# val-iisc/Reflecting-Reality

Measured on AMD Instinct MI355X. Metric: images/sec at 512x512, 50-step DDIM, SD1.5+BrushNet, higher is better.
Workload: dtype bf16; 1 GPU; SD1.5 + BrushNet(6 cond ch) depth-cond inpaint, batch 4x512x512 per GPU, 50-step DDIM, CFG 7.5, VAE encode+decode included, random-init weights, inputs resident on the device; per_gpu_batch=4, global_batch=4, height=512, width=512, denoise_steps=50, parallelism=batch-shard x1 (no collective)

## Files before the change

### reflecting-reality_amd/csrc/gemm_conv_kernel.h

```cpp
#pragma once
#include "mf_common.h"

#include <type_traits>

#ifndef MF_XTAP
#define MF_XTAP 1
#endif
#ifndef MF_AEARLY
#define MF_AEARLY 1
#endif

namespace mfgemm {

static __device__ __attribute__((aligned(16))) unsigned int g_zero_page[16];

#ifdef MF_STAMPS
#define MF_STAMP(slot) do { if (p.stamps) { const int t_ = (int)threadIdx.x; \
    if (t_ == 0) p.stamps[(size_t)blockIdx.x * 32 + (slot)] = __builtin_amdgcn_s_memrealtime(); \
    else if (t_ == (int)blockDim.x - 256) p.stamps[(size_t)blockIdx.x * 32 + 16 + (slot)] = __builtin_amdgcn_s_memrealtime(); } } while (0)
#define MF_STAMP_DRAIN() asm volatile("s_waitcnt vmcnt(0)" ::: "memory")
#define MF_CLK(v) const unsigned long long v = __builtin_amdgcn_s_memtime()
#define MF_SUM(acc, a, b) acc += (b) - (a)
#define MF_PUT(slot, v) do { if (p.stamps) { const int t_ = (int)threadIdx.x; \
    if (t_ == 0) p.stamps[(size_t)blockIdx.x * 32 + (slot)] = (v); \
    else if (t_ == (int)blockDim.x - 256) p.stamps[(size_t)blockIdx.x * 32 + 16 + (slot)] = (v); } } while (0)
#else
#define MF_STAMP(slot) do { } while (0)
#define MF_STAMP_DRAIN() do { } while (0)
#define MF_CLK(v) do { } while (0)
#define MF_SUM(acc, a, b) do { } while (0)
#define MF_PUT(slot, v) do { } while (0)
#endif

struct GemmArgs {
    const char* a0; const char* a1;
    int C0, Ctot;
    int ld0b, ld1b;
    int Hin, Win, Ho, Wo, HoWo, KW, stride, pad_t, pad_l, ups;
    const char* w; int64_t ldw;
    int M, N, K;
    int zdiv; int64_t a_zs_o, a_zs_i, w_zs_o, w_zs_i, o_zs_o, o_zs_i;
    int splitk, kt_per_split, nkt, nz;
    float* ws;
    unsigned* sk_tickets;
    const float* bias; int bias_mode;
    const float* rs; const float* cs; int64_t rs_zs, cs_zs;
    const float* temb; int64_t ld_temb;
    const char* res0; int res0_dt; int64_t ld_res0;
    const char* res1; int res1_dt; int64_t ld_res1;
    int res1_rows;
    float alpha; int act;
    char* out; int out_dt; int64_t ldc;
    int tiles_n, tiles_m, ord_mfast, ord_pw, nblk, vec_ok, fast, dbg_no_res_pre;
    int dbg_epi;
    int pointwise;
    int howo_sh, wo_sh, ho_sh;
    unsigned wfr_magic;
    int epb;
    int epb_sh;
// ... 94 lines not shown
    if (p.act == MF_ACT_SILU) {
#pragma unroll
        for (int j = 0; j < 8; ++j) v[j] = silu_precise(v[j]);
    }
    if (p.act == MF_ACT_GEGLU4) {
        float g[4];
        if (p.out_dt != MF_F32) {
#pragma unroll
            for (int j = 0; j < 4; ++j) {
                const float x = v[4 + j];
                const float z = fabsf(x) * 0.70710678118654752440f;
                const float t = __builtin_amdgcn_rcpf(fmaf(0.3275911f, z, 1.0f));
                const float poly = t * fmaf(t, fmaf(t, fmaf(t, fmaf(t, 1.061405429f, -1.453152027f), 1.421413741f), -0.284496736f), 0.254829592f);
                const float e = 1.0f - poly * __builtin_amdgcn_exp2f(-z * z * 1.44269504088896340736f);
                g[j] = v[j] * (0.5f * x + 0.5f * fabsf(x) * e);
            }
        } else {
#pragma unroll
            for (int j = 0; j < 4; ++j) g[j] = v[j] * (0.5f * v[4 + j] * (1.0f + erff(v[4 + j] * 0.70710678118654752440f)));
        }
        const int64_t o = zo + (int64_t)m * p.ldc + (n >> 1);
        if (p.out_dt == MF_F32) {
            *reinterpret_cast<float4*>(p.out + o * 4) = make_float4(g[0], g[1], g[2], g[3]);
        } else {
            uint2 u;
            u.x = pack_h2<F16>(g[0], g[1]);
            u.y = pack_h2<F16>(g[2], g[3]);
            *reinterpret_cast<uint2*>(p.out + o * 2) = u;
        }
        return;
    }
    const int64_t o = zo + (int64_t)m * p.ldc + n;
    if (p.out_dt == MF_F32) {
        *reinterpret_cast<float4*>(p.out + o * 4) = make_float4(v[0], v[1], v[2], v[3]);
        *reinterpret_cast<float4*>(p.out + o * 4 + 16) = make_float4(v[4], v[5], v[6], v[7]);
    } else {
        *reinterpret_cast<uint4*>(p.out + o * 2) = pack_h8<F16>(v);
    }
}

__device__ __forceinline__ uint4 ld8f_to_bf16(const char* p) {
    const float4 lo = *reinterpret_cast<const float4*>(p);
    const float4 hi = *reinterpret_cast<const float4*>(p + 16);
    uint4 r;
    r.x = pack_bf16x2(lo.x, lo.y);
    r.y = pack_bf16x2(lo.z, lo.w);
    r.z = pack_bf16x2(hi.x, hi.y);
    r.w = pack_bf16x2(hi.z, hi.w);
    return r;
}

typedef __attribute__((address_space(1))) const void* gbl_ptr_t;

__device__ __forceinline__ void dma16(const char* src, char* lds_wave_base) {
    const unsigned lds_off = __builtin_amdgcn_readfirstlane((unsigned)(size_t)(lds_ptr_t)lds_wave_base);
    unsigned keep;
    asm volatile("s_mov_b32 %0, m0\n\ts_mov_b32 m0, %2\n\ts_nop 0\n\tglobal_load_lds_dwordx4 %1, off\n\ts_mov_b32 m0, %0"
                 : "=&s"(keep) : "v"(src), "s"(lds_off) : "memory");
}

template <int DT>
__device__ __forceinline__ f32x4_t mfma16x32(bf16x8_t a, bf16x8_t b, f32x4_t c, int, int, int) {
    if constexpr (DT == MF_F16) return __builtin_amdgcn_mfma_f32_16x16x32_f16(__builtin_bit_cast(f16x8_t, a), __builtin_bit_cast(f16x8_t, b), c, 0, 0, 0);
    else return __builtin_amdgcn_mfma_f32_16x16x32_bf16(a, b, c, 0, 0, 0);
}
template <int DT>
__device__ __forceinline__ f32x16_t mfma32x16(bf16x8_t a, bf16x8_t b, f32x16_t c) {
    if constexpr (DT == MF_F16) return __builtin_amdgcn_mfma_f32_32x32x16_f16(__builtin_bit_cast(f16x8_t, a), __builtin_bit_cast(f16x8_t, b), c, 0, 0, 0);
    else return __builtin_amdgcn_mfma_f32_32x32x16_bf16(a, b, c, 0, 0, 0);
}

#define MF_FX_XT 1
#define MF_FX_EPB 2
#define MF_FX_AE 4
#define MF_FX_ALL 7
#define MF_FX_XQ 8

constexpr int epb_pitch(int bn) { return (bn + 63) / 64 * 64; }
constexpr int epb_off(int bm, int bn, int stages, bool dx, bool ws) {
    return dx ? 2 * (bm + 32) * 128 + (ws ? stages : 2) * bn * 128 : stages * (bm + bn) * 128 + (ws ? bm * 8 : 0);
}
constexpr int epb_nimg(int bm, int bn, int stages, bool dx, bool ws) {
    if (!ws) return 0;
    const int room = 160 * 1024 - epb_off(bm, bn, stages, dx, ws), row = epb_pitch(bn) * 4;
    return room >= 6 * row ? 4 : (room >= 3 * row ? 1 : 0);
}

constexpr int min_waves(int bm, int bn, int stages, int nthr) {
    const int smem = stages * (bm + bn) * 128;
    int blocks = 160 * 1024 / smem;
    if (blocks > 8) blocks = 8;
    int w = blocks * (nthr / 64) / 4;
    return w < 1 ? 1 : (w > 4 ? 4 : w);
}

template <int BM, int BN, int NT_ALL, bool F16>
__device__ __forceinline__ void splitk_combine_tail(const GemmArgs& p, char* smem, int tile_m, int tile_n, int z, int zq, int64_t zo, int t) {
    asm volatile("s_waitcnt vmcnt(0)" ::: "memory");
    __syncthreads();
    unsigned* last_flag = reinterpret_cast<unsigned*>(smem);
    if (t == 0) {
        __builtin_amdgcn_fence(__ATOMIC_RELEASE, "agent");
        asm volatile("s_waitcnt vmcnt(0)" ::: "memory");
        unsigned* tk = p.sk_tickets + ((int64_t)z * p.tiles_m + tile_m) * p.tiles_n + tile_n;
        const unsigned prev = __hip_atomic_fetch_add(tk, 1u, __ATOMIC_RELAXED, __HIP_MEMORY_SCOPE_AGENT);
        const bool last = prev == (unsigned)p.splitk - 1u;
// ... 298 lines not shown
    auto store_tile_regs = [&](int stage) {
        char* As = smem + stage * STAGE_BYTES + tid * 16;
        char* Bs = As + BM * 128;
#pragma unroll
        for (int i = 0; i < (A_F32 ? A_IT : 1); ++i) *reinterpret_cast<uint4*>(As + i * RPP * 128) = ra[i];
#pragma unroll
        for (int i = 0; i < (A_F32 ? B_IT : 1); ++i) *reinterpret_cast<uint4*>(Bs + i * RPP * 128) = rb[i];
    };

    f32x16_t acc[MT][NT];
#pragma unroll
    for (int i = 0; i < MT; ++i)
#pragma unroll
        for (int j = 0; j < NT; ++j)
#pragma unroll
            for (int e = 0; e < 16; ++e) acc[i][j][e] = 0.0f;
    f32x4_t acc16[P16 ? MT16 : 1][P16 ? NT16 : 1];
#pragma unroll
    for (int a = 0; a < (P16 ? MT16 : 1); ++a)
#pragma unroll
        for (int b = 0; b < (P16 ? NT16 : 1); ++b) acc16[a][b] = f32x4_t{0.0f, 0.0f, 0.0f, 0.0f};

    const int frow = lane & 31;
    const int fh = lane >> 5;
    const int fkey = (frow >> 1) & 7;

    float split_amax = 0.0f;
    auto split8 = [&](const uint4& c0, const uint4& c1, uint4& hi, uint4& lo) {
        const float x[8] = {__uint_as_float(c0.x), __uint_as_float(c0.y), __uint_as_float(c0.z), __uint_as_float(c0.w),
                            __uint_as_float(c1.x), __uint_as_float(c1.y), __uint_as_float(c1.z), __uint_as_float(c1.w)};
        if constexpr (DT == MF_F16X3) {
#pragma unroll
            for (int e = 0; e < 4; ++e) split_amax = mf_amax3(split_amax, x[2 * e], x[2 * e + 1]);
        }
        unsigned h[4], l[4];
#pragma unroll
        for (int e = 0; e < 4; ++e) {
            if constexpr (X1) {
                h[e] = pack_bf16x2(x[2 * e], x[2 * e + 1]);
                l[e] = 0;
            } else if constexpr (DT == MF_F16X3) {
                mf_split_f16x2(x[2 * e], x[2 * e + 1], h[e], l[e]);
            } else {
                const unsigned ua = __float_as_uint(x[2 * e]), ub = __float_as_uint(x[2 * e + 1]);
                h[e] = (ua >> 16) | (ub & 0xffff0000u);
                l[e] = pack_bf16x2(x[2 * e] - __uint_as_float(ua & 0xffff0000u), x[2 * e + 1] - __uint_as_float(ub & 0xffff0000u));
            }
        }
        hi = uint4{h[0], h[1], h[2], h[3]};
        lo = uint4{l[0], l[1], l[2], l[3]};
    };
    auto mma16 = [&](const uint4& a, const uint4& b, f32x16_t& c) {
        if constexpr (DT == MF_F16X3)
            c = __builtin_amdgcn_mfma_f32_32x32x16_f16(__builtin_bit_cast(f16x8_t, a), __builtin_bit_cast(f16x8_t, b), c, 0, 0, 0);
        else
            c = __builtin_amdgcn_mfma_f32_32x32x16_bf16(__builtin_bit_cast(bf16x8_t, a), __builtin_bit_cast(bf16x8_t, b), c, 0, 0, 0);
    };
    auto compute_split = [&](const char* const (&Ap)[MT], const int (&Ak)[MT], const char* Bp) {
        if constexpr (FP8) {
#pragma unroll
            for (int ks = 0; ks < 2; ++ks) {
                i32x8_t fa[MT], fb[NT];
#pragma unroll
                for (int i = 0; i < MT; ++i) {
                    const uint4 c0 = *reinterpret_cast<const uint4*>(Ap[i] + (((4 * ks + 2 * fh) ^ Ak[i]) << 4));
                    const uint4 c1 = *reinterpret_cast<const uint4*>(Ap[i] + (((4 * ks + 2 * fh + 1) ^ Ak[i]) << 4));
                    fa[i] = i32x8_t{(int)c0.x, (int)c0.y, (int)c0.z, (int)c0.w, (int)c1.x, (int)c1.y, (int)c1.z, (int)c1.w};
                }
#pragma unroll
                for (int j = 0; j < NT; ++j) {
                    const uint4 c0 = *reinterpret_cast<const uint4*>(Bp + j * 32 * 128 + (((4 * ks + 2 * fh) ^ fkey) << 4));
                    const uint4 c1 = *reinterpret_cast<const uint4*>(Bp + j * 32 * 128 + (((4 * ks + 2 * fh + 1) ^ fkey) << 4));
                    fb[j] = i32x8_t{(int)c0.x, (int)c0.y, (int)c0.z, (int)c0.w, (int)c1.x, (int)c1.y, (int)c1.z, (int)c1.w};
                }
#pragma unroll
                for (int i = 0; i < MT; ++i)
#pragma unroll
                    for (int j = 0; j < NT; ++j)
                        acc[i][j] = __builtin_amdgcn_mfma_scale_f32_32x32x64_f8f6f4(fa[i], fb[j], acc[i][j], 0, 0, 0, 0x7f7f7f7f, 0, 0x7f7f7f7f);
            }
            return;
        }
#pragma unroll
        for (int ks = 0; ks < 2; ++ks) {
            uint4 ah[MT], al[MT], bh[NT], bl[NT];
#pragma unroll
            for (int i = 0; i < MT; ++i) {
                const uint4 c0 = *reinterpret_cast<const uint4*>(Ap[i] + (((4 * ks + 2 * fh) ^ Ak[i]) << 4));
                const uint4 c1 = *reinterpret_cast<const uint4*>(Ap[i] + (((4 * ks + 2 * fh + 1) ^ Ak[i]) << 4));
                split8(c0, c1, ah[i], al[i]);
            }
#pragma unroll
            for (int j = 0; j < NT; ++j) {
                if constexpr (WPK) {
                    bh[j] = *reinterpret_cast<const uint4*>(Bp + j * 32 * 128 + (((2 * ks + fh) ^ fkey) << 4));
                    bl[j] = *reinterpret_cast<const uint4*>(Bp + j * 32 * 128 + (((4 + 2 * ks + fh) ^ fkey) << 4));
                } else {
                    const uint4 c0 = *reinterpret_cast<const uint4*>(Bp + j * 32 * 128 + (((4 * ks + 2 * fh) ^ fkey) << 4));
                    const uint4 c1 = *reinterpret_cast<const uint4*>(Bp + j * 32 * 128 + (((4 * ks + 2 * fh + 1) ^ fkey) << 4));
                    split8(c0, c1, bh[j], bl[j]);
                }
            }
#pragma unroll
            for (int i = 0; i < MT; ++i)
#pragma unroll
                for (int j = 0; j < NT; ++j) {
                    if constexpr (!X1) {
                        mma16(al[i], bh[j], acc[i][j]);
                        mma16(ah[i], bl[j], acc[i][j]);
                    }
                    mma16(ah[i], bh[j], acc[i][j]);
                }
        }
    };

    const int r16 = lane & 15, kg = lane >> 4;
    auto compute_m16 = [&](const char* const (&Ap)[2 * MT], const int (&Ak)[2 * MT], const char* Bp) {
        const int key16 = (r16 >> 1) & 7;
        uint4 fa[2][2 * MT], fb[2][2 * NT];
#pragma unroll
        for (int ks = 0; ks < 2; ++ks) {
#pragma unroll
            for (int t = 0; t < 2 * MT; ++t) fa[ks][t] = *reinterpret_cast<const uint4*>(Ap[t] + (((4 * ks + kg) ^ Ak[t]) << 4));
#pragma unroll
            for (int t = 0; t < 2 * NT; ++t) fb[ks][t] = *reinterpret_cast<const uint4*>(Bp + t * 16 * 128 + (((4 * ks + kg) ^ key16) << 4));
        }
#pragma unroll
        for (int ks = 0; ks < 2; ++ks)
#pragma unroll
            for (int i = 0; i < MT; ++i)
#pragma unroll
                for (int j = 0; j < NT; ++j)
#pragma unroll
                    for (int q = 0; q < 4; ++q) {
                        f32x4_t c = {acc[i][j][4 * q], acc[i][j][4 * q + 1], acc[i][j][4 * q + 2], acc[i][j][4 * q + 3]};
                        c = mfma16x32<DT>(__builtin_bit_cast(bf16x8_t, fa[ks][2 * i + (q >> 1)]),
                                                                    __builtin_bit_cast(bf16x8_t, fb[ks][2 * j + (q & 1)]), c, 0, 0, 0);
                        acc[i][j][4 * q] = c[0]; acc[i][j][4 * q + 1] = c[1]; acc[i][j][4 * q + 2] = c[2]; acc[i][j][4 * q + 3] = c[3];
                    }
    };

    auto mma = [&](const uint4 (&fa)[MT], const uint4 (&fb)[NT]) {
#pragma unroll
        for (int i = 0; i < MT; ++i)
#pragma unroll
            for (int j = 0; j < NT; ++j) {
                if constexpr (DT == MF_BF16) {
                    acc[i][j] = __builtin_amdgcn_mfma_f32_32x32x16_bf16(
                        __builtin_bit_cast(bf16x8_t, fa[i]), __builtin_bit_cast(bf16x8_t, fb[j]), acc[i][j], 0, 0, 0);
                } else if constexpr (DT == MF_F16) {
                    acc[i][j] = __builtin_amdgcn_mfma_f32_32x32x16_f16(
                        __builtin_bit_cast(f16x8_t, fa[i]), __builtin_bit_cast(f16x8_t, fb[j]), acc[i][j], 0, 0, 0);
                } else {
                    const f32x4_t av = __builtin_bit_cast(f32x4_t, fa[i]);
                    const f32x4_t bv = __builtin_bit_cast(f32x4_t, fb[j]);
#pragma unroll
                    for (int e = 0; e < 4; ++e)
                        acc[i][j] = __builtin_amdgcn_mfma_f32_32x32x2f32(av[e], bv[e], acc[i][j], 0, 0, 0);
                }
            }
    };
    auto compute = [&](int stage) {
        if constexpr (P16) {
            const char* A16 = smem + stage * STAGE_BYTES + (wm * WM + r16) * 128;
            const char* B16 = smem + stage * STAGE_BYTES + BM * 128 + (wn * WN + r16) * 128;
            const int key16 = (r16 >> 1) & 7;
            uint4 fa[2][MT16], fb[2][NT16];
#pragma unroll
            for (int ks = 0; ks < 2; ++ks) {
#pragma unroll
                for (int t = 0; t < MT16; ++t) fa[ks][t] = *reinterpret_cast<const uint4*>(A16 + t * 16 * 128 + (((4 * ks + kg) ^ key16) << 4));
#pragma unroll
                for (int b = 0; b < NT16; ++b) fb[ks][b] = *reinterpret_cast<const uint4*>(B16 + b * 16 * 128 + (((4 * ks + kg) ^ key16) << 4));
            }
#pragma unroll
            for (int ks = 0; ks < 2; ++ks)
#pragma unroll
                for (int a = 0; a < MT16; ++a)
#pragma unroll
                    for (int b = 0; b < NT16; ++b)
                        acc16[a][b] = mfma16x32<DT>(__builtin_bit_cast(bf16x8_t, fa[ks][a]),
                                                                              __builtin_bit_cast(bf16x8_t, fb[ks][b]), acc16[a][b], 0, 0, 0);
            return;
        }
        const char* As = smem + stage * STAGE_BYTES + (wm * WM + frow) * 128;
        const char* Bs = smem + stage * STAGE_BYTES + BM * 128 + (wn * WN + frow) * 128;
        if constexpr (SPLIT || FP8) {
            const char* Ap[MT]; int Ak[MT];
#pragma unroll
            for (int i = 0; i < MT; ++i) { Ap[i] = As + i * 32 * 128; Ak[i] = fkey; }
            compute_split(Ap, Ak, Bs);
            return;
        }
        if constexpr (M16) {
            const char* A16 = smem + stage * STAGE_BYTES + (wm * WM + r16) * 128;
            const char* B16 = smem + stage * STAGE_BYTES + BM * 128 + (wn * WN + r16) * 128;
            const char* Ap[2 * MT]; int Ak[2 * MT];
#pragma unroll
            for (int t = 0; t < 2 * MT; ++t) { Ap[t] = A16 + t * 16 * 128; Ak[t] = (r16 >> 1) & 7; }
            compute_m16(Ap, Ak, B16);
            return;
        }
        uint4 fa0[MT], fb0[NT], fa1[MT], fb1[NT];
        auto ldfrag = [&](int ks, uint4 (&fa)[MT], uint4 (&fb)[NT]) {
            const int coff = (((2 * ks + fh) ^ fkey) << 4);
#pragma unroll
            for (int i = 0; i < MT; ++i) fa[i] = *reinterpret_cast<const uint4*>(As + i * 32 * 128 + coff);
#pragma unroll
            for (int j = 0; j < NT; ++j) fb[j] = *reinterpret_cast<const uint4*>(Bs + j * 32 * 128 + coff);
        };
        ldfrag(0, fa0, fb0);
        ldfrag(1, fa1, fb1);
        __builtin_amdgcn_sched_barrier(0);
        mma(fa0, fb0);
        __builtin_amdgcn_sched_barrier(0);
        ldfrag(2, fa0, fb0);
        __builtin_amdgcn_sched_barrier(0);
        mma(fa1, fb1);
        __builtin_amdgcn_sched_barrier(0);
        ldfrag(3, fa1, fb1);
        __builtin_amdgcn_sched_barrier(0);
        mma(fa0, fb0);
        mma(fa1, fb1);
    };

    constexpr bool XQ = (FX & MF_FX_XQ) != 0 && WS && H16 && !A_F32 && !M16 && !P16;
    constexpr bool XT = XQ || ((FX & MF_FX_XT) != 0 && WS && H16 && !A_F32 && (MF_XTAP != 0) && !(WAVES_M == 8 && WAVES_N == 1));
    constexpr int XNA = !XT ? 1 : XQ ? MT : (P16 ? MT16 : 2 * MT), XNB = !XT ? 1 : XQ ? NT : (P16 ? NT16 : 2 * NT);
    uint4 xa[2][XNA], xb[2][XNB];
    auto xt_load = [&](auto S, auto P, const char* Ab, auto arow, const char* Bb) {
        constexpr int ss = decltype(S)::value, hh = decltype(P)::value;
        if constexpr (XQ) {
            const int ch = 2 * hh + fh;
#pragma unroll
            for (int i = 0; i < MT; ++i) {
                const int r = arow(i);
                xa[ss][i] = *reinterpret_cast<const uint4*>(Ab + r * 128 + ((ch ^ ((r >> 1) & 7)) << 4));
            }
#pragma unroll
            for (int j = 0; j < NT; ++j) xb[ss][j] = *reinterpret_cast<const uint4*>(Bb + j * 32 * 128 + ((ch ^ fkey) << 4));
        } else if constexpr (P16 || M16) {
            const int key16 = (r16 >> 1) & 7;
#pragma unroll
            for (int t = 0; t < XNA; ++t) {
                const int r = arow(t);
                xa[ss][t] = *reinterpret_cast<const uint4*>(Ab + r * 128 + (((4 * hh + kg) ^ ((r >> 1) & 7)) << 4));
            }
#pragma unroll
            for (int t = 0; t < XNB; ++t) xb[ss][t] = *reinterpret_cast<const uint4*>(Bb + t * 16 * 128 + (((4 * hh + kg) ^ key16) << 4));
        } else {
#pragma unroll
            for (int kk = 0; kk < 2; ++kk) {
                const int ch = 2 * (2 * hh + kk) + fh;
#pragma unroll
                for (int i = 0; i < MT; ++i) {
                    const int r = arow(i);
                    xa[ss][kk * MT + i] = *reinterpret_cast<const uint4*>(Ab + r * 128 + ((ch ^ ((r >> 1) & 7)) << 4));
                }
#pragma unroll
                for (int j = 0; j < NT; ++j) xb[ss][kk * NT + j] = *reinterpret_cast<const uint4*>(Bb + j * 32 * 128 + ((ch ^ fkey) << 4));
            }
        }
    };
    auto xt_mma = [&](auto S) {
        constexpr int hh = decltype(S)::value;
        if constexpr (XQ) {
#pragma unroll
            for (int i = 0; i < MT; ++i)
#pragma unroll
                for (int j = 0; j < NT; ++j)
                    acc[i][j] = mfma32x16<DT>(__builtin_bit_cast(bf16x8_t, xa[hh][i]), __builtin_bit_cast(bf16x8_t, xb[hh][j]), acc[i][j]);
        } else if constexpr (P16) {
#pragma unroll
            for (int a = 0; a < MT16; ++a)
#pragma unroll
                for (int b = 0; b < NT16; ++b)
                    acc16[a][b] = mfma16x32<DT>(__builtin_bit_cast(bf16x8_t, xa[hh][a]),
                                                                          __builtin_bit_cast(bf16x8_t, xb[hh][b]), acc16[a][b], 0, 0, 0);
        } else if constexpr (M16) {
#pragma unroll
            for (int i = 0; i < MT; ++i)
#pragma unroll
                for (int j = 0; j < NT; ++j)
#pragma unroll
                    for (int q = 0; q < 4; ++q) {
                        f32x4_t c = {acc[i][j][4 * q], acc[i][j][4 * q + 1], acc[i][j][4 * q + 2], acc[i][j][4 * q + 3]};
                        c = mfma16x32<DT>(__builtin_bit_cast(bf16x8_t, xa[hh][2 * i + (q >> 1)]),
                                                                    __builtin_bit_cast(bf16x8_t, xb[hh][2 * j + (q & 1)]), c, 0, 0, 0);
                        acc[i][j][4 * q] = c[0]; acc[i][j][4 * q + 1] = c[1]; acc[i][j][4 * q + 2] = c[2]; acc[i][j][4 * q + 3] = c[3];
                    }
        } else {
#pragma unroll
            for (int kk = 0; kk < 2; ++kk)
#pragma unroll
                for (int i = 0; i < MT; ++i)
#pragma unroll
                    for (int j = 0; j < NT; ++j)
                        acc[i][j] = mfma32x16<DT>(__builtin_bit_cast(bf16x8_t, xa[hh][kk * MT + i]), __builtin_bit_cast(bf16x8_t, xb[hh][kk * NT + j]), acc[i][j]);
        }
    };
    using H0 = std::integral_constant<int, 0>;
    using H1 = std::integral_constant<int, 1>;
    using H2 = std::integral_constant<int, 2>;
    using H3 = std::integral_constant<int, 3>;
    auto xt_loop = [&](auto&& ld, auto&& adv) {
        auto head = [&]() {
            ld(H1{}, H1{});
            __builtin_amdgcn_sched_barrier(0);
            xt_mma(H0{});
            __builtin_amdgcn_sched_barrier(0);
            if constexpr (XQ) {
                ld(H0{}, H2{});
                __builtin_amdgcn_sched_barrier(0);
                xt_mma(H1{});
                __builtin_amdgcn_sched_barrier(0);
                ld(H1{}, H3{});
                __builtin_amdgcn_sched_barrier(0);
                xt_mma(H0{});
                __builtin_amdgcn_sched_barrier(0);
            }
        };
        ld(H0{}, H0{});
        [[maybe_unused]] unsigned long long w_bar = 0;
        MF_CLK(tl0);
        for (int t = 0; t + 1 < nt; ++t) {
            head();
            adv();
            __builtin_amdgcn_s_waitcnt(0xc07f);
            MF_CLK(tb0);
            __builtin_amdgcn_s_barrier();
            MF_CLK(tb1);
            MF_SUM(w_bar, tb0, tb1);
            ld(H0{}, H0{});
            __builtin_amdgcn_sched_barrier(0);
            xt_mma(H1{});
            __builtin_amdgcn_sched_barrier(0);
        }
        head();
        xt_mma(H1{});
        MF_CLK(tl1);
        MF_PUT(13, w_bar); MF_PUT(14, tl1 - tl0); MF_PUT(15, (unsigned long long)nt);
    };

    MF_STAMP(1);
    if (nt > 0) {
        if constexpr (DXR) {
            static_assert(!A_F32 && (WS ? STAGES == 3 : STAGES == 2), "dx reuse: DMA staging; W ring 2 deep, 3 when WS (a 4-deep ring measured no faster)");
            constexpr int WST = WS ? STAGES : 2;
            constexpr int AROWS = BM + RPP, A3_IT = AROWS / RPP;
            constexpr int AB = AROWS * 128, WB = BN * 128;
            static_assert(WAVES_M * WAVES_N * SR * EP_RS <= 2 * AB + WST * WB, "epilogue slabs must fit in this loop's LDS");
// ... 54 lines not shown
#pragma unroll
                for (int i = 0; i < B_IT; ++i) dma16_buf(w3[i] + wk, sW, lb + i * RPP * 128);
                if (AE && i_kx == 2 && i_tap + 1 < nt) {
                    int n_cg = i_cg + 1, n_ky = i_ky;
                    if (n_cg == nck) { n_cg = 0; ++n_ky; }
                    issue_a(n_ky, n_cg, i_grp + 1);
                }
                ++i_tap;
                if (++i_kx == 3) {
                    i_kx = 0; ++i_grp;
                    if (++i_cg == nck) { i_cg = 0; ++i_ky; }
                }
            };
            int arow0[MT];
#pragma unroll
            for (int i = 0; i < MT; ++i) {
                const int m = wm * WM + i * 32 + frow;
                const int ir = p.wo_sh >= 0 ? m >> weff_sh : m / weff;
                arow0[i] = ir * wfr + (m - ir * weff);
            }
            int arow16[2 * MT];
#pragma unroll
            for (int t = 0; t < 2 * MT; ++t) {
                const int m = wm * WM + t * 16 + r16;
                const int ir = p.wo_sh >= 0 ? m >> weff_sh : m / weff;
                arow16[t] = ir * wfr + (m - ir * weff);
            }
            auto compute3 = [&](int abuf, int wstage, int kx) {
                const char* Ab = smem + abuf * AB;
                if constexpr (P16) {
                    const char* Bp = smem + 2 * AB + wstage * WB + (wn * WN + r16) * 128;
                    const int key16 = (r16 >> 1) & 7;
                    const char* Ap[MT16]; int Ak[MT16];
#pragma unroll
                    for (int t = 0; t < MT16; ++t) {
                        const int r = arow16[t] + kx;
                        Ap[t] = Ab + r * 128;
                        Ak[t] = (r >> 1) & 7;
                    }
                    uint4 fa[2][MT16], fb[2][NT16];
#pragma unroll
                    for (int ks = 0; ks < 2; ++ks) {
#pragma unroll
                        for (int t = 0; t < MT16; ++t) fa[ks][t] = *reinterpret_cast<const uint4*>(Ap[t] + (((4 * ks + kg) ^ Ak[t]) << 4));
#pragma unroll
                        for (int b = 0; b < NT16; ++b) fb[ks][b] = *reinterpret_cast<const uint4*>(Bp + b * 16 * 128 + (((4 * ks + kg) ^ key16) << 4));
                    }
#pragma unroll
                    for (int ks = 0; ks < 2; ++ks)
#pragma unroll
                        for (int a = 0; a < MT16; ++a)
#pragma unroll
                            for (int b = 0; b < NT16; ++b)
                                acc16[a][b] = mfma16x32<DT>(__builtin_bit_cast(bf16x8_t, fa[ks][a]),
                                                                                      __builtin_bit_cast(bf16x8_t, fb[ks][b]), acc16[a][b], 0, 0, 0);
                    return;
                }
                const char* Bs = smem + 2 * AB + wstage * WB + (wn * WN + frow) * 128;
                if constexpr (M16) {
                    const char* Ap[2 * MT]; int Ak[2 * MT];
#pragma unroll
                    for (int t = 0; t < 2 * MT; ++t) {
                        const int r = arow16[t] + kx;
                        Ap[t] = Ab + r * 128;
                        Ak[t] = (r >> 1) & 7;
                    }
                    compute_m16(Ap, Ak, smem + 2 * AB + wstage * WB + (wn * WN + r16) * 128);
                    return;
                }
                int aoffs[MT], akey[MT];
#pragma unroll
                for (int i = 0; i < MT; ++i) {
                    const int r = arow0[i] + kx;
                    aoffs[i] = r * 128;
                    akey[i] = (r >> 1) & 7;
                }
                if constexpr (SPLIT || FP8) {
                    const char* Ap[MT];
#pragma unroll
                    for (int i = 0; i < MT; ++i) Ap[i] = Ab + aoffs[i];
                    compute_split(Ap, akey, Bs);
                    return;
                }
                uint4 fa0[MT], fb0[NT], fa1[MT], fb1[NT];
                auto ldfrag = [&](int ks, uint4 (&fa)[MT], uint4 (&fb)[NT]) {
                    const int cb = (((2 * ks + fh) ^ fkey) << 4);
#pragma unroll
                    for (int i = 0; i < MT; ++i)
                        fa[i] = *reinterpret_cast<const uint4*>(Ab + aoffs[i] + (((2 * ks + fh) ^ akey[i]) << 4));
#pragma unroll
                    for (int j = 0; j < NT; ++j) fb[j] = *reinterpret_cast<const uint4*>(Bs + j * 32 * 128 + cb);
                };
                ldfrag(0, fa0, fb0);
                ldfrag(1, fa1, fb1);
                __builtin_amdgcn_sched_barrier(0);
                mma(fa0, fb0);
                __builtin_amdgcn_sched_barrier(0);
                ldfrag(2, fa0, fb0);
                __builtin_amdgcn_sched_barrier(0);
                mma(fa1, fb1);
                __builtin_amdgcn_sched_barrier(0);
                ldfrag(3, fa1, fb1);
                __builtin_amdgcn_sched_barrier(0);
                mma(fa0, fb0);
                mma(fa1, fb1);
            };
            if constexpr (WS) {
                constexpr int PFD = WST - 1;
// ... 189 lines not shown
                            if constexpr (P16 || M16) xt_load(S, P, Ab, [&](int t) { return arb + t * 16; }, Bb);
                            else xt_load(S, P, Ab, [&](int i) { return arb + i * 32; }, Bb);
                        };
                        xt_loop(ld, [&]() { st_c = st_c == STAGES - 1 ? 0 : st_c + 1; });
                    } else
                    for (int t = 0; t < nt; ++t) {
                        compute(st_c);
                        st_c = st_c == STAGES - 1 ? 0 : st_c + 1;
                        if (t + 1 < nt) __builtin_amdgcn_s_barrier();
                    }
                }
            };
            if constexpr (WS) {
                if (p.fast) {
                    if (producer) fast_init();
                    ring_ws(issue_tile_fast);
                } else {
                    ring_ws(issue_tile);
                }
            } else if (p.fast) {
                fast_init();
                ring(issue_tile_fast);
            } else {
                ring(issue_tile);
            }
        } else {
            load_tile_regs();
            store_tile_regs(0);
            if (nt > 1) load_tile_regs();
            __syncthreads();
            for (int t = 0; t < nt; ++t) {
                compute(t & 1);
                if (t + 1 < nt) {
                    store_tile_regs((t + 1) & 1);
                    if (t + 2 < nt) load_tile_regs();
                }
                __syncthreads();
            }
        }
    }
    MF_STAMP(3);
    if constexpr (EPB_NIMG > 0) {
        if (producer && epb) wait_vmcnt<0>();
    }
    __syncthreads();
    MF_STAMP(4);
    if constexpr (DT == MF_F16X3) mf_raise_if_over(p.ovf, split_amax);

    char* slab = smem + wave * (SR * EP_RS);
    constexpr int CPR = WN / 8;
    constexpr int ITEMS = SR * CPR;
    float* ws = p.splitk > 1 ? p.ws + ((int64_t)ksplit * p.nz + z) * (int64_t)p.M * p.N : nullptr;
    const int64_t zo = zq * p.o_zs_o + zr * p.o_zs_i;
    const bool res_pre = !ws && p.vec_ok && (p.res0 || p.res1) && (!p.res0 || p.res0_dt != MF_F32) &&
                         (!p.res1 || p.res1_dt != MF_F32) && !p.dbg_no_res_pre;
    constexpr int NIT = (ITEMS + 63) / 64;
    if constexpr (WS) {
        constexpr int NCW = WAVES_M * WAVES_N, TW = NCW + 4, NCHUNK = NCW * NIT, MAXC = (NCHUNK + TW - 1) / TW;
        const int g = producer ? NCW + wave : wave;
        const bool gn = p.gn_part != nullptr;
        constexpr int GNP = (NCW * WN + TW * 64 - 1) / (TW * 64);
        float gns[GNP], gnq[GNP];
#pragma unroll
        for (int k = 0; k < GNP; ++k) { gns[k] = 0.0f; gnq[k] = 0.0f; }
#pragma unroll
        for (int ih = 0; ih < MT * (32 / SR); ++ih) {
            const int i = ih / (32 / SR), half = ih % (32 / SR);
            uint4 q0[MAXC], q1[MAXC];
            auto coords = [&](int u, int& sw, int& row, int& ec, int& m, int& n) -> bool {
                const int c = g + u * TW;
                sw = c / NIT;
                const int it = (c - sw * NIT) * 64 + lane;
                row = it / CPR; ec = (it - row * CPR) * 8;
                const int swm = sw / WAVES_N, swn = sw - swm * WAVES_N;
                m = m0 + swm * WM + i * 32 + half * SR + row;
                n = n0 + swn * WN + ec;
                return c < NCHUNK && (ITEMS % 64 == 0 || it < ITEMS);
            };
            if (res_pre) {
#pragma unroll
                for (int u = 0; u < MAXC; ++u) {
                    int sw, row, ec, m, n;
                    const bool on = coords(u, sw, row, ec, m, n);
                    q0[u] = uint4{0, 0, 0, 0}; q1[u] = uint4{0, 0, 0, 0};
                    if (on && m < p.M && n + 8 <= p.N) {
                        if (p.res0) q0[u] = *reinterpret_cast<const uint4*>(p.res0 + ((int64_t)m * p.ld_res0 + n) * 2);
                        if (p.res1) q1[u] = *reinterpret_cast<const uint4*>(p.res1 + ((int64_t)res1_row(p, m) * p.ld_res1 + n) * 2);
                    }
                }
            }
            if (!producer) {
                if constexpr (P16) {
#pragma unroll
                    for (int a = 0; a < 2; ++a)
#pragma unroll
                        for (int b = 0; b < NT16; ++b)
#pragma unroll
                            for (int r = 0; r < 4; ++r) {
                                const int row = 16 * a + 4 * kg + r - half * SR;
                                if (SR == 32 || a == half)
                                    *reinterpret_cast<float*>(slab + row * EP_RS + (16 * b + r16) * 4) = acc16[2 * i + a][b][r];
                            }
                } else {
#pragma unroll
                    for (int j = 0; j < NT; ++j)
#pragma unroll
                        for (int e = half * (SR / 2); e < half * (SR / 2) + SR / 2; ++e) {
                            if constexpr (M16) {
                                const int row = 16 * (e >> 3) + 4 * kg + (e & 3) - half * SR;
                                *reinterpret_cast<float*>(slab + row * EP_RS + (j * 32 + 16 * ((e >> 2) & 1) + r16) * 4) = acc[i][j][e];
                            } else {
                                const int row = (e & 3) + 8 * (e >> 2) + 4 * fh - half * SR;
                                *reinterpret_cast<float*>(slab + row * EP_RS + (j * 32 + frow) * 4) = acc[i][j][e];
                            }
                        }
                }
            }
            MF_STAMP(7 + 3 * ih);
            __builtin_amdgcn_s_waitcnt(0xc07f);
            __builtin_amdgcn_s_barrier();
            MF_STAMP(8 + 3 * ih);
#pragma unroll
            for (int u = 0; u < MAXC; ++u) {
                int sw, row, ec, m, n;
                if (!coords(u, sw, row, ec, m, n)) continue;
                const char* sl = smem + sw * (SR * EP_RS);
                const float2* lnst = reinterpret_cast<const float2*>(smem + STAGES * STAGE_BYTES);
                if (p.vt_out && n0 + (sw % WAVES_N) * WN >= p.vt_n0) {
                    static_assert(SR % 8 == 0 && (SR / 8) * WN == ITEMS, "transposed items cover the slab");
                    const int c = g + u * TW, it = (c - sw * NIT) * 64 + lane;
                    const int rg = it % (SR / 8), col = it / (SR / 8);
                    const int swm = sw / WAVES_N, swn = sw - swm * WAVES_N;
                    const int mt = m0 + swm * WM + i * 32 + half * SR + rg * 8, nt_ = n0 + swn * WN + col;
                    if (mt < p.M && nt_ < p.N) {
                        float tv[8];
#pragma unroll
                        for (int j = 0; j < 8; ++j) tv[j] = *reinterpret_cast<const float*>(sl + (rg * 8 + j) * EP_RS + col * 4);
                        const char* erow = smem + EPB_OFF + (nt_ - n0) * 4;
                        if (p.ln_cs) {
                            const float cs = epb ? *reinterpret_cast<const float*>(erow + EPB_PITCH * 4) : p.ln_cs[nt_];
#pragma unroll
                            for (int j = 0; j < 8; ++j) {
                                const float2 st = lnst[mt - m0 + j];
                                tv[j] = st.y * (tv[j] - st.x * cs);
                            }
                        }
                        const float b = p.bias ? (epb ? *reinterpret_cast<const float*>(erow) : p.bias[nt_]) : 0.0f;
#pragma unroll
                        for (int j = 0; j < 8; ++j) tv[j] = (tv[j] + b) * p.alpha;
                        const int img = mt / p.vt_tokens, tok = mt - img * p.vt_tokens;
                        const uint4 o = pack_h8<DT == MF_F16>(tv);
                        *reinterpret_cast<uint4*>(p.vt_out + (((int64_t)img * (p.N - p.vt_n0) + (nt_ - p.vt_n0)) * p.vt_ld + tok) * 2) = o;
                    }
                    continue;
                }
                float v[8];
                float4 lo, hi;
#ifdef MF_STAMPS
                if (p.dbg_epi & 2) { lo = make_float4(1.0f, 2.0f, 3.0f, (float)u); hi = lo; } else
#endif
                {
                    lo = *reinterpret_cast<const float4*>(sl + row * EP_RS + ec * 4);
                    hi = *reinterpret_cast<const float4*>(sl + row * EP_RS + ec * 4 + 16);
                }
#ifdef MF_STAMPS
                if (p.dbg_epi & 1) { asm volatile("" ::"v"(lo.x), "v"(hi.w)); continue; }
#endif
                if (p.ln_cs && m < p.M && n + 8 <= p.N) {
                    const float2 st = lnst[m - m0];
                    const float* lc = epb ? reinterpret_cast<const float*>(smem + EPB_OFF + (EPB_PITCH + n - n0) * 4) : p.ln_cs + n;
                    const float4 c0 = *reinterpret_cast<const float4*>(lc);
                    const float4 c1 = *reinterpret_cast<const float4*>(lc + 4);
                    lo.x = st.y * (lo.x - st.x * c0.x); lo.y = st.y * (lo.y - st.x * c0.y);
                    lo.z = st.y * (lo.z - st.x * c0.z); lo.w = st.y * (lo.w - st.x * c0.w);
                    hi.x = st.y * (hi.x - st.x * c1.x); hi.y = st.y * (hi.y - st.x * c1.y);
                    hi.z = st.y * (hi.z - st.x * c1.z); hi.w = st.y * (hi.w - st.x * c1.w);
                }
                v[0] = lo.x; v[1] = lo.y; v[2] = lo.z; v[3] = lo.w; v[4] = hi.x; v[5] = hi.y; v[6] = hi.z; v[7] = hi.w;
                if (m < p.M && n < p.N) {
                    if (ws) {
                        if (n + 8 <= p.N && (p.N & 3) == 0) {
                            *reinterpret_cast<float4*>(ws + (int64_t)m * p.N + n) = lo;
                            *reinterpret_cast<float4*>(ws + (int64_t)m * p.N + n + 4) = hi;
                        } else {
                            for (int jj = 0; jj < 8 && n + jj < p.N; ++jj) ws[(int64_t)m * p.N + n + jj] = v[jj];
                        }
                    } else if (p.vec_ok && n + 8 <= p.N) {
                        if (epb) {
                            const char* eb = smem + EPB_OFF + (n - n0) * 4;
                            epilogue_store8<DT == MF_F16>(p, zo, m, n, v, res_pre, q0[u], q1[u], zq, eb, eb + (2 + (m >> p.epb_sh) - (m0 >> p.epb_sh)) * (EPB_PITCH * 4));
                        } else {
                            epilogue_store8<DT == MF_F16>(p, zo, m, n, v, res_pre, q0[u], q1[u], zq);
                        }
                        if (gn) {
                            char* slw = smem + sw * (SR * EP_RS) + row * EP_RS + ec * 4;
                            *reinterpret_cast<float4*>(slw) = make_float4(v[0], v[1], v[2], v[3]);
                            *reinterpret_cast<float4*>(slw + 16) = make_float4(v[4], v[5], v[6], v[7]);
                        }
                    } else {
                        for (int jj = 0; jj < 8 && n + jj < p.N; ++jj) epilogue_store(p, zo, m, n + jj, v[jj], zq);
                    }
                }
            }
            MF_STAMP(9 + 3 * ih);
            if (gn) {
                __builtin_amdgcn_s_waitcnt(0xc07f);
                __builtin_amdgcn_s_barrier();
#pragma unroll
                for (int k = 0; k < GNP; ++k) {
                    const int pid = (g + k * TW) * 64 + lane;
                    if (pid < NCW * WN) {
                        const int sw = pid / WN, col = pid - sw * WN;
                        const char* sl = smem + sw * (SR * EP_RS) + col * 4;
                        float a = 0.0f, b = 0.0f;
#pragma unroll
                        for (int r = 0; r < SR; ++r) {
                            const float x = *reinterpret_cast<const float*>(sl + r * EP_RS);
                            a += x; b = fmaf(x, x, b);
                        }
                        gns[k] += a; gnq[k] += b;
                    }
                }
            }
            if (ih + 1 < MT * (32 / SR) || gn) {
                __builtin_amdgcn_s_waitcnt(0xc07f);
                __builtin_amdgcn_s_barrier();
            }
        }
        if (gn) {
            float2* red = reinterpret_cast<float2*>(smem);
#pragma unroll
            for (int k = 0; k < GNP; ++k) {
                const int pid = (g + k * TW) * 64 + lane;
                if (pid < NCW * WN) {
                    const int sw = pid / WN, col = pid - sw * WN;
                    const int swm = sw / WAVES_N, swn = sw - swm * WAVES_N;
// ... 3 lines not shown
            __builtin_amdgcn_s_waitcnt(0xc07f);
            __builtin_amdgcn_s_barrier();
            const int tcol = (int)threadIdx.x;
            float a = 0.0f, b = 0.0f;
            if (tcol < BN && n0 + tcol < p.N) {
#pragma unroll
                for (int w2 = 0; w2 < WAVES_M; ++w2) { const float2 x = red[w2 * BN + tcol]; a += x.x; b += x.y; }
                p.gn_part[(int64_t)tile_m * p.N + n0 + tcol] = make_float2(a, b);
            }
            if (p.gn_grp) {
                float2* tot = red + WAVES_M * BN;
                if (tcol < BN) tot[tcol] = make_float2(a, b);
                __builtin_amdgcn_s_waitcnt(0xc07f);
                __builtin_amdgcn_s_barrier();
                const int cpg = p.gn_cpg, c0g = tcol * cpg;
                if (c0g < BN && n0 + c0g < p.N) {
                    float ga = 0.0f, gb = 0.0f;
                    for (int j = 0; j < cpg; ++j) { const float2 x = tot[c0g + j]; ga += x.x; gb += x.y; }
                    p.gn_grp[(int64_t)tile_m * (p.N / cpg) + (n0 + c0g) / cpg] = make_float2(ga, gb);
                }
            }
        }
        MF_STAMP_DRAIN();
        MF_STAMP(5);
        if constexpr (SKF) {
            if (ws) splitk_combine_tail<BM, BN, NTHR + 256, DT == MF_F16>(p, smem, tile_m, tile_n, z, zq, zo, (int)threadIdx.x);
        }
        MF_STAMP(6);
        return;
    }
    const bool gn = p.gn_part != nullptr;
    constexpr int GNC = (WN + 63) / 64;
    float gns[GNC], gnq[GNC];
#pragma unroll
    for (int k = 0; k < GNC; ++k) { gns[k] = 0.0f; gnq[k] = 0.0f; }
#pragma unroll
    for (int ih = 0; ih < MT * (32 / SR); ++ih) {
        const int i = ih / (32 / SR), half = ih % (32 / SR);
        uint4 q0[NIT], q1[NIT];
        if (res_pre) {
#pragma unroll
            for (int k = 0; k < NIT; ++k) {
                const int it = k * 64 + lane;
                const int row = it / CPR, ec = (it - row * CPR) * 8;
                const int m = m0 + wm * WM + i * 32 + half * SR + row;
                const int n = n0 + wn * WN + ec;
                q0[k] = uint4{0, 0, 0, 0}; q1[k] = uint4{0, 0, 0, 0};
                if ((ITEMS % 64 == 0 || it < ITEMS) && m < p.M && n + 8 <= p.N) {
                    if (p.res0) q0[k] = *reinterpret_cast<const uint4*>(p.res0 + ((int64_t)m * p.ld_res0 + n) * 2);
                    if (p.res1) q1[k] = *reinterpret_cast<const uint4*>(p.res1 + ((int64_t)res1_row(p, m) * p.ld_res1 + n) * 2);
                }
            }
        }
        if constexpr (P16) {
#pragma unroll
            for (int a = 0; a < 2; ++a)
#pragma unroll
                for (int b = 0; b < NT16; ++b)
#pragma unroll
                    for (int r = 0; r < 4; ++r) {
                        const int row = 16 * a + 4 * kg + r - half * SR;
                        if (SR == 32 || a == half)
                            *reinterpret_cast<float*>(slab + row * EP_RS + (16 * b + r16) * 4) = acc16[2 * i + a][b][r];
                    }
        } else
#pragma unroll
        for (int j = 0; j < NT; ++j)
#pragma unroll
            for (int e = half * (SR / 2); e < half * (SR / 2) + SR / 2; ++e) {
                if constexpr (M16) {
                    const int row = 16 * (e >> 3) + 4 * kg + (e & 3) - half * SR;
                    *reinterpret_cast<float*>(slab + row * EP_RS + (j * 32 + 16 * ((e >> 2) & 1) + r16) * 4) = acc[i][j][e];
                } else {
                    const int row = (e & 3) + 8 * (e >> 2) + 4 * fh - half * SR;
                    *reinterpret_cast<float*>(slab + row * EP_RS + (j * 32 + frow) * 4) = acc[i][j][e];
                }
            }
        __builtin_amdgcn_s_waitcnt(0xc07f);
        __builtin_amdgcn_wave_barrier();
#pragma unroll
        for (int it0 = 0; it0 < ITEMS; it0 += 64) {
            const int it = it0 + lane;
            if (ITEMS % 64 != 0 && it >= ITEMS) continue;
            const int row = it / CPR, ec = (it - row * CPR) * 8;
            const int m = m0 + wm * WM + i * 32 + half * SR + row;
            const int n = n0 + wn * WN + ec;
            float v[8];
            const float4 lo = *reinterpret_cast<const float4*>(slab + row * EP_RS + ec * 4);
            const float4 hi = *reinterpret_cast<const float4*>(slab + row * EP_RS + ec * 4 + 16);
            v[0] = lo.x; v[1] = lo.y; v[2] = lo.z; v[3] = lo.w; v[4] = hi.x; v[5] = hi.y; v[6] = hi.z; v[7] = hi.w;
            if (m < p.M && n < p.N) {
                if (ws) {
                    if (n + 8 <= p.N && (p.N & 3) == 0) {
                        *reinterpret_cast<float4*>(ws + (int64_t)m * p.N + n) = lo;
                        *reinterpret_cast<float4*>(ws + (int64_t)m * p.N + n + 4) = hi;
                    } else {
                        for (int jj = 0; jj < 8 && n + jj < p.N; ++jj) ws[(int64_t)m * p.N + n + jj] = v[jj];
                    }
                } else if (p.vec_ok && n + 8 <= p.N) {
                    epilogue_store8<DT == MF_F16>(p, zo, m, n, v, res_pre, q0[it0 / 64], q1[it0 / 64], zq);
                    if (gn) {
                        *reinterpret_cast<float4*>(slab + row * EP_RS + ec * 4) = make_float4(v[0], v[1], v[2], v[3]);
                        *reinterpret_cast<float4*>(slab + row * EP_RS + ec * 4 + 16) = make_float4(v[4], v[5], v[6], v[7]);
                    }
                } else {
                    for (int jj = 0; jj < 8 && n + jj < p.N; ++jj) epilogue_store(p, zo, m, n + jj, v[jj], zq);
                }
            }
        }
        __builtin_amdgcn_s_waitcnt(0xc07f);
        __builtin_amdgcn_wave_barrier();
        if (gn) {
#pragma unroll
            for (int k = 0; k < GNC; ++k) {
                const int col = lane + 64 * k;
                if (WN % 64 == 0 || col < WN) {
                    float a = 0.0f, b = 0.0f;
#pragma unroll
                    for (int r = 0; r < SR; ++r) {
                        const float x = *reinterpret_cast<const float*>(slab + r * EP_RS + col * 4);
                        a += x; b = fmaf(x, x, b);
                    }
                    gns[k] += a; gnq[k] += b;
                }
            }
            __builtin_amdgcn_s_waitcnt(0xc07f);
            __builtin_amdgcn_wave_barrier();
        }
    }
    if (gn) {
        __syncthreads();
        float2* red = reinterpret_cast<float2*>(smem);
#pragma unroll
        for (int k = 0; k < GNC; ++k) {
            const int col = lane + 64 * k;
            if (WN % 64 == 0 || col < WN) red[wm * BN + wn * WN + col] = make_float2(gns[k], gnq[k]);
        }
        __syncthreads();
        float2* tot = red + WAVES_M * BN;
        for (int tcol = (int)threadIdx.x; tcol < BN; tcol += NTHR) {
            float a = 0.0f, b = 0.0f;
            if (n0 + tcol < p.N) {
#pragma unroll
                for (int w2 = 0; w2 < WAVES_M; ++w2) { const float2 x = red[w2 * BN + tcol]; a += x.x; b += x.y; }
                p.gn_part[(int64_t)tile_m * p.N + n0 + tcol] = make_float2(a, b);
            }
            if (p.gn_grp) tot[tcol] = make_float2(a, b);
        }
// ... 68 lines not shown
```

Baseline: 5.314 images/sec.

## Transpose MFMA operand order to vectorize epilogue slab writes; buffer-store split-K workspace

Every MFMA call now takes the B operand first and A second, so the accumulator holds the transposed tile and each lane owns four consecutive output columns. The epilogue then writes the accumulators to the LDS slab as 16-byte float4 stores instead of scalar stores, using a permlane16 swap for the half-slab case, and the scalar loops are folded into a shared slab_write lambda. Split-K workspace stores go through buffer-resource b128 stores, with an optional write-through cache flag that is off by default. The gain is fewer LDS store instructions in the epilogue; the risk is that the new lane-to-row/column mapping must exactly match the transposed accumulator layout across every variant (P16, M16, FP8, f32).

New measurement: 5.321 images/sec, median of 6. About the same (+0.1%).

```diff
diff --git a/reflecting-reality_amd/csrc/gemm_conv_kernel.h b/reflecting-reality_amd/csrc/gemm_conv_kernel.h
--- a/reflecting-reality_amd/csrc/gemm_conv_kernel.h
+++ b/reflecting-reality_amd/csrc/gemm_conv_kernel.h
@@ -5,6 +5,9 @@
 
 #ifndef MF_XTAP
 #define MF_XTAP 1
+#endif
+#ifndef MF_WS_WT
+#define MF_WS_WT 0
 #endif
 #ifndef MF_AEARLY
 #define MF_AEARLY 1
@@ -205,6 +208,12 @@
 
 typedef __attribute__((address_space(1))) const void* gbl_ptr_t;
 
+typedef __attribute__((ext_vector_type(4))) unsigned mf_u32x4_t;
+__device__ __forceinline__ void store16_wt(__amdgpu_buffer_rsrc_t rsrc, unsigned byte_off, const float4& v) {
+    const mf_u32x4_t w = {__float_as_uint(v.x), __float_as_uint(v.y), __float_as_uint(v.z), __float_as_uint(v.w)};
+    __builtin_amdgcn_raw_buffer_store_b128(w, rsrc, (int)byte_off, 0, MF_WS_WT ? 16 : 0);
+}
+
 __device__ __forceinline__ void dma16(const char* src, char* lds_wave_base) {
     const unsigned lds_off = __builtin_amdgcn_readfirstlane((unsigned)(size_t)(lds_ptr_t)lds_wave_base);
     unsigned keep;
@@ -609,9 +618,9 @@
     };
     auto mma16 = [&](const uint4& a, const uint4& b, f32x16_t& c) {
         if constexpr (DT == MF_F16X3)
-            c = __builtin_amdgcn_mfma_f32_32x32x16_f16(__builtin_bit_cast(f16x8_t, a), __builtin_bit_cast(f16x8_t, b), c, 0, 0, 0);
+            c = __builtin_amdgcn_mfma_f32_32x32x16_f16(__builtin_bit_cast(f16x8_t, b), __builtin_bit_cast(f16x8_t, a), c, 0, 0, 0);
         else
-            c = __builtin_amdgcn_mfma_f32_32x32x16_bf16(__builtin_bit_cast(bf16x8_t, a), __builtin_bit_cast(bf16x8_t, b), c, 0, 0, 0);
+            c = __builtin_amdgcn_mfma_f32_32x32x16_bf16(__builtin_bit_cast(bf16x8_t, b), __builtin_bit_cast(bf16x8_t, a), c, 0, 0, 0);
     };
     auto compute_split = [&](const char* const (&Ap)[MT], const int (&Ak)[MT], const char* Bp) {
         if constexpr (FP8) {
@@ -634,7 +643,7 @@
                 for (int i = 0; i < MT; ++i)
 #pragma unroll
                     for (int j = 0; j < NT; ++j)
-                        acc[i][j] = __builtin_amdgcn_mfma_scale_f32_32x32x64_f8f6f4(fa[i], fb[j], acc[i][j], 0, 0, 0, 0x7f7f7f7f, 0, 0x7f7f7f7f);
+                        acc[i][j] = __builtin_amdgcn_mfma_scale_f32_32x32x64_f8f6f4(fb[j], fa[i], acc[i][j], 0, 0, 0, 0x7f7f7f7f, 0, 0x7f7f7f7f);
             }
             return;
         }
@@ -691,8 +700,8 @@
 #pragma unroll
                     for (int q = 0; q < 4; ++q) {
                         f32x4_t c = {acc[i][j][4 * q], acc[i][j][4 * q + 1], acc[i][j][4 * q + 2], acc[i][j][4 * q + 3]};
-                        c = mfma16x32<DT>(__builtin_bit_cast(bf16x8_t, fa[ks][2 * i + (q >> 1)]),
-                                                                    __builtin_bit_cast(bf16x8_t, fb[ks][2 * j + (q & 1)]), c, 0, 0, 0);
+                        c = mfma16x32<DT>(__builtin_bit_cast(bf16x8_t, fb[ks][2 * j + (q & 1)]),
+                                                                    __builtin_bit_cast(bf16x8_t, fa[ks][2 * i + (q >> 1)]), c, 0, 0, 0);
                         acc[i][j][4 * q] = c[0]; acc[i][j][4 * q + 1] = c[1]; acc[i][j][4 * q + 2] = c[2]; acc[i][j][4 * q + 3] = c[3];
                     }
     };
@@ -704,16 +713,16 @@
             for (int j = 0; j < NT; ++j) {
                 if constexpr (DT == MF_BF16) {
                     acc[i][j] = __builtin_amdgcn_mfma_f32_32x32x16_bf16(
-                        __builtin_bit_cast(bf16x8_t, fa[i]), __builtin_bit_cast(bf16x8_t, fb[j]), acc[i][j], 0, 0, 0);
+                        __builtin_bit_cast(bf16x8_t, fb[j]), __builtin_bit_cast(bf16x8_t, fa[i]), acc[i][j], 0, 0, 0);
                 } else if constexpr (DT == MF_F16) {
                     acc[i][j] = __builtin_amdgcn_mfma_f32_32x32x16_f16(
-                        __builtin_bit_cast(f16x8_t, fa[i]), __builtin_bit_cast(f16x8_t, fb[j]), acc[i][j], 0, 0, 0);
+                        __builtin_bit_cast(f16x8_t, fb[j]), __builtin_bit_cast(f16x8_t, fa[i]), acc[i][j], 0, 0, 0);
                 } else {
                     const f32x4_t av = __builtin_bit_cast(f32x4_t, fa[i]);
                     const f32x4_t bv = __builtin_bit_cast(f32x4_t, fb[j]);
 #pragma unroll
                     for (int e = 0; e < 4; ++e)
-                        acc[i][j] = __builtin_amdgcn_mfma_f32_32x32x2f32(av[e], bv[e], acc[i][j], 0, 0, 0);
+                        acc[i][j] = __builtin_amdgcn_mfma_f32_32x32x2f32(bv[e], av[e], acc[i][j], 0, 0, 0);
                 }
             }
     };
@@ -736,8 +745,8 @@
                 for (int a = 0; a < MT16; ++a)
 #pragma unroll
                     for (int b = 0; b < NT16; ++b)
-                        acc16[a][b] = mfma16x32<DT>(__builtin_bit_cast(bf16x8_t, fa[ks][a]),
-                                                                              __builtin_bit_cast(bf16x8_t, fb[ks][b]), acc16[a][b], 0, 0, 0);
+                        acc16[a][b] = mfma16x32<DT>(__builtin_bit_cast(bf16x8_t, fb[ks][b]),
+                                                                              __builtin_bit_cast(bf16x8_t, fa[ks][a]), acc16[a][b], 0, 0, 0);
             return;
         }
         const char* As = smem + stage * STAGE_BYTES + (wm * WM + frow) * 128;
@@ -826,14 +835,14 @@
             for (int i = 0; i < MT; ++i)
 #pragma unroll
                 for (int j = 0; j < NT; ++j)
-                    acc[i][j] = mfma32x16<DT>(__builtin_bit_cast(bf16x8_t, xa[hh][i]), __builtin_bit_cast(bf16x8_t, xb[hh][j]), acc[i][j]);
+                    acc[i][j] = mfma32x16<DT>(__builtin_bit_cast(bf16x8_t, xb[hh][j]), __builtin_bit_cast(bf16x8_t, xa[hh][i]), acc[i][j]);
         } else if constexpr (P16) {
 #pragma unroll
             for (int a = 0; a < MT16; ++a)
 #pragma unroll
                 for (int b = 0; b < NT16; ++b)
-                    acc16[a][b] = mfma16x32<DT>(__builtin_bit_cast(bf16x8_t, xa[hh][a]),
-                                                                          __builtin_bit_cast(bf16x8_t, xb[hh][b]), acc16[a][b], 0, 0, 0);
+                    acc16[a][b] = mfma16x32<DT>(__builtin_bit_cast(bf16x8_t, xb[hh][b]),
+                                                                          __builtin_bit_cast(bf16x8_t, xa[hh][a]), acc16[a][b], 0, 0, 0);
         } else if constexpr (M16) {
 #pragma unroll
             for (int i = 0; i < MT; ++i)
@@ -842,8 +851,8 @@
 #pragma unroll
                     for (int q = 0; q < 4; ++q) {
                         f32x4_t c = {acc[i][j][4 * q], acc[i][j][4 * q + 1], acc[i][j][4 * q + 2], acc[i][j][4 * q + 3]};
-                        c = mfma16x32<DT>(__builtin_bit_cast(bf16x8_t, xa[hh][2 * i + (q >> 1)]),
-                                                                    __builtin_bit_cast(bf16x8_t, xb[hh][2 * j + (q & 1)]), c, 0, 0, 0);
+                        c = mfma16x32<DT>(__builtin_bit_cast(bf16x8_t, xb[hh][2 * j + (q & 1)]),
+                                                                    __builtin_bit_cast(bf16x8_t, xa[hh][2 * i + (q >> 1)]), c, 0, 0, 0);
                         acc[i][j][4 * q] = c[0]; acc[i][j][4 * q + 1] = c[1]; acc[i][j][4 * q + 2] = c[2]; acc[i][j][4 * q + 3] = c[3];
                     }
         } else {
@@ -853,7 +862,7 @@
                 for (int i = 0; i < MT; ++i)
 #pragma unroll
                     for (int j = 0; j < NT; ++j)
-                        acc[i][j] = mfma32x16<DT>(__builtin_bit_cast(bf16x8_t, xa[hh][kk * MT + i]), __builtin_bit_cast(bf16x8_t, xb[hh][kk * NT + j]), acc[i][j]);
+                        acc[i][j] = mfma32x16<DT>(__builtin_bit_cast(bf16x8_t, xb[hh][kk * NT + j]), __builtin_bit_cast(bf16x8_t, xa[hh][kk * MT + i]), acc[i][j]);
         }
     };
     using H0 = std::integral_constant<int, 0>;
@@ -1014,8 +1023,8 @@
                         for (int a = 0; a < MT16; ++a)
 #pragma unroll
                             for (int b = 0; b < NT16; ++b)
-                                acc16[a][b] = mfma16x32<DT>(__builtin_bit_cast(bf16x8_t, fa[ks][a]),
-                                                                                      __builtin_bit_cast(bf16x8_t, fb[ks][b]), acc16[a][b], 0, 0, 0);
+                                acc16[a][b] = mfma16x32<DT>(__builtin_bit_cast(bf16x8_t, fb[ks][b]),
+                                                                                      __builtin_bit_cast(bf16x8_t, fa[ks][a]), acc16[a][b], 0, 0, 0);
                     return;
                 }
                 const char* Bs = smem + 2 * AB + wstage * WB + (wn * WN + frow) * 128;
@@ -1311,9 +1320,51 @@
     constexpr int ITEMS = SR * CPR;
     float* ws = p.splitk > 1 ? p.ws + ((int64_t)ksplit * p.nz + z) * (int64_t)p.M * p.N : nullptr;
     const int64_t zo = zq * p.o_zs_o + zr * p.o_zs_i;
+    const bool ws_vec = (p.N & 3) == 0 && (int64_t)p.M * p.N < (int64_t)1 << 30;
+    const __amdgpu_buffer_rsrc_t ws_rsrc = __builtin_amdgcn_make_buffer_rsrc(ws, 0, ws_vec ? p.M * p.N * 4 : 0, 0x00020000);
     const bool res_pre = !ws && p.vec_ok && (p.res0 || p.res1) && (!p.res0 || p.res0_dt != MF_F32) &&
                          (!p.res1 || p.res1_dt != MF_F32) && !p.dbg_no_res_pre;
     constexpr int NIT = (ITEMS + 63) / 64;
+    static_assert(EP_RS % 16 == 0, "16-byte slab writes");
+    auto slab_write = [&](int i, int half) {
+        if constexpr (P16) {
+#pragma unroll
+            for (int a = 0; a < 2; ++a)
+#pragma unroll
+                for (int b = 0; b < NT16; ++b)
+                    if (SR == 32 || a == half) {
+                        const f32x4_t c = acc16[2 * i + a][b];
+                        *reinterpret_cast<float4*>(slab + (16 * a + r16 - half * SR) * EP_RS + (16 * b + 4 * kg) * 4) = make_float4(c[0], c[1], c[2], c[3]);
+                    }
+        } else {
+#pragma unroll
+            for (int j = 0; j < NT; ++j)
+#pragma unroll
+                for (int q = 0; q < 4; ++q) {
+                    const float4 c = make_float4(acc[i][j][4 * q], acc[i][j][4 * q + 1], acc[i][j][4 * q + 2], acc[i][j][4 * q + 3]);
+                    if constexpr (M16) {
+                        if (SR == 32 || (q >> 1) == half)
+                            *reinterpret_cast<float4*>(slab + (16 * (q >> 1) + r16 - half * SR) * EP_RS + (j * 32 + 16 * (q & 1) + 4 * kg) * 4) = c;
+                    } else if constexpr (SR == 32) {
+                        *reinterpret_cast<float4*>(slab + frow * EP_RS + (j * 32 + 8 * q + 4 * fh) * 4) = c;
+                    } else {
+                        if (half == 0 && q < 2) {
+#pragma unroll
+                            for (int r = 0; r < 4; ++r) {
+                                const auto x = __builtin_amdgcn_permlane16_swap(__float_as_uint(acc[i][j][4 * q + r]), __float_as_uint(acc[i][j][4 * q + r + 8]), false, false);
+                                acc[i][j][4 * q + r] = __uint_as_float(x[0]);
+                                acc[i][j][4 * q + r + 8] = __uint_as_float(x[1]);
+                            }
+                        }
+                        if (q < 2) {
+                            const int e0 = 4 * (2 * half + q);
+                            *reinterpret_cast<float4*>(slab + (frow & 15) * EP_RS + (j * 32 + 8 * (q + 2 * (frow >> 4)) + 4 * fh) * 4) =
+                                make_float4(acc[i][j][e0], acc[i][j][e0 + 1], acc[i][j][e0 + 2], acc[i][j][e0 + 3]);
+                        }
+                    }
+                }
+        }
+    };
     if constexpr (WS) {
         constexpr int NCW = WAVES_M * WAVES_N, TW = NCW + 4, NCHUNK = NCW * NIT, MAXC = (NCHUNK + TW - 1) / TW;
         const int g = producer ? NCW + wave : wave;
@@ -1348,33 +1399,7 @@
                     }
                 }
             }
-            if (!producer) {
-                if constexpr (P16) {
-#pragma unroll
-                    for (int a = 0; a < 2; ++a)
-#pragma unroll
-                        for (int b = 0; b < NT16; ++b)
-#pragma unroll
-                            for (int r = 0; r < 4; ++r) {
-                                const int row = 16 * a + 4 * kg + r - half * SR;
-                                if (SR == 32 || a == half)
-                                    *reinterpret_cast<float*>(slab + row * EP_RS + (16 * b + r16) * 4) = acc16[2 * i + a][b][r];
-                            }
-                } else {
-#pragma unroll
-                    for (int j = 0; j < NT; ++j)
-#pragma unroll
-                        for (int e = half * (SR / 2); e < half * (SR / 2) + SR / 2; ++e) {
-                            if constexpr (M16) {
-                                const int row = 16 * (e >> 3) + 4 * kg + (e & 3) - half * SR;
-                                *reinterpret_cast<float*>(slab + row * EP_RS + (j * 32 + 16 * ((e >> 2) & 1) + r16) * 4) = acc[i][j][e];
-                            } else {
-                                const int row = (e & 3) + 8 * (e >> 2) + 4 * fh - half * SR;
-                                *reinterpret_cast<float*>(slab + row * EP_RS + (j * 32 + frow) * 4) = acc[i][j][e];
-                            }
-                        }
-                }
-            }
+            if (!producer) slab_write(i, half);
             MF_STAMP(7 + 3 * ih);
             __builtin_amdgcn_s_waitcnt(0xc07f);
             __builtin_amdgcn_s_barrier();
@@ -1438,9 +1463,9 @@
                 v[0] = lo.x; v[1] = lo.y; v[2] = lo.z; v[3] = lo.w; v[4] = hi.x; v[5] = hi.y; v[6] = hi.z; v[7] = hi.w;
                 if (m < p.M && n < p.N) {
                     if (ws) {
-                        if (n + 8 <= p.N && (p.N & 3) == 0) {
-                            *reinterpret_cast<float4*>(ws + (int64_t)m * p.N + n) = lo;
-                            *reinterpret_cast<float4*>(ws + (int64_t)m * p.N + n + 4) = hi;
+                        if (n + 8 <= p.N && ws_vec) {
+                            store16_wt(ws_rsrc, (unsigned)(m * p.N + n) * 4u, lo);
+                            store16_wt(ws_rsrc, (unsigned)(m * p.N + n) * 4u + 16u, hi);
                         } else {
                             for (int jj = 0; jj < 8 && n + jj < p.N; ++jj) ws[(int64_t)m * p.N + n + jj] = v[jj];
                         }
@@ -1550,30 +1575,7 @@
                 }
             }
         }
-        if constexpr (P16) {
-#pragma unroll
-            for (int a = 0; a < 2; ++a)
-#pragma unroll
-                for (int b = 0; b < NT16; ++b)
-#pragma unroll
-                    for (int r = 0; r < 4; ++r) {
-                        const int row = 16 * a + 4 * kg + r - half * SR;
-                        if (SR == 32 || a == half)
-                            *reinterpret_cast<float*>(slab + row * EP_RS + (16 * b + r16) * 4) = acc16[2 * i + a][b][r];
-                    }
-        } else
-#pragma unroll
-        for (int j = 0; j < NT; ++j)
-#pragma unroll
-            for (int e = half * (SR / 2); e < half * (SR / 2) + SR / 2; ++e) {
-                if constexpr (M16) {
-                    const int row = 16 * (e >> 3) + 4 * kg + (e & 3) - half * SR;
-                    *reinterpret_cast<float*>(slab + row * EP_RS + (j * 32 + 16 * ((e >> 2) & 1) + r16) * 4) = acc[i][j][e];
-                } else {
-                    const int row = (e & 3) + 8 * (e >> 2) + 4 * fh - half * SR;
-                    *reinterpret_cast<float*>(slab + row * EP_RS + (j * 32 + frow) * 4) = acc[i][j][e];
-                }
-            }
+        slab_write(i, half);
         __builtin_amdgcn_s_waitcnt(0xc07f);
         __builtin_amdgcn_wave_barrier();
 #pragma unroll
@@ -1589,9 +1591,9 @@
             v[0] = lo.x; v[1] = lo.y; v[2] = lo.z; v[3] = lo.w; v[4] = hi.x; v[5] = hi.y; v[6] = hi.z; v[7] = hi.w;
             if (m < p.M && n < p.N) {
                 if (ws) {
-                    if (n + 8 <= p.N && (p.N & 3) == 0) {
-                        *reinterpret_cast<float4*>(ws + (int64_t)m * p.N + n) = lo;
-                        *reinterpret_cast<float4*>(ws + (int64_t)m * p.N + n + 4) = hi;
+                    if (n + 8 <= p.N && ws_vec) {
+                        store16_wt(ws_rsrc, (unsigned)(m * p.N + n) * 4u, lo);
+                        store16_wt(ws_rsrc, (unsigned)(m * p.N + n) * 4u + 16u, hi);
                     } else {
                         for (int jj = 0; jj < 8 && n + jj < p.N; ++jj) ws[(int64_t)m * p.N + n + jj] = v[jj];
                     }
```
